# Russoul/cuda-mat

Measured on AMD Instinct MI355X. Metric: BiCGSTAB iters/sec + SpMV effective HBM GB/s, 10M-row CSR at 1/2/4/8 GPUs, higher is better.
Workload: dtype f64

## Files before the change

### cuda_mat_amd/csrc/config.cpp

```cpp
#include "config.h"

#include <stdio.h>
#include <stdlib.h>
#include <string.h>

#include <unistd.h>

#include <mutex>
#include <set>
#include <string>

extern char **environ;

#include "common.h"

namespace cm {

namespace {

enum Kind { K_FLAG, K_INT, K_LLONG, K_ENUM, K_FAIL };

struct Option {
    const char *name;
    Kind kind;
    int Config::*field;
    long long Config::*wide;
    long long lo, hi;
    const char *words;
    const char *help;
};

#define OPT_FLAG(NAME, FIELD, HELP) {NAME, K_FLAG, &Config::FIELD, nullptr, 0, 1, nullptr, HELP}
#define OPT_INT(NAME, FIELD, LO, HI, HELP) {NAME, K_INT, &Config::FIELD, nullptr, LO, HI, nullptr, HELP}
#define OPT_ENUM(NAME, FIELD, WORDS, HELP) {NAME, K_ENUM, &Config::FIELD, nullptr, 0, 0, WORDS, HELP}

const Option kOptions[] = {
    OPT_INT("VERBOSE", verbose, 0, 2, "1: set-up breakdowns and auto-tune timings on stderr; 2: also the memory classes of a large blocked copy's arrays (timed probe, diagnosis)"),
    OPT_FLAG("ROCTX", roctx, "roctx ranges around solver creation, SpMV-form choice, ILU(0) set-up, the loop, SpMVs and all-reduces"),
    OPT_ENUM("SPMV_MODE", spmv_mode, "csr=0,pb=1,sell=2,pat=3", "force the CSR forms / the blocked two-phase form / SELL-C-sigma / the row-pattern dictionary"),
    OPT_FLAG("SPMV_SELL", spmv_sell, "0: keep SELL-C-sigma out of the candidates"),
    OPT_ENUM("SPMV_FORM", spmv_form, "lanes=1,tiles=2", "inside the CSR forms: lanes per row / nnz-balanced tiles"),
    OPT_INT("SPMV_LANES", spmv_lanes, 2, 64, "lanes per row, a power of two (and no stream tiles)"),
    OPT_FLAG("SPMV_COMPRESS", spmv_compress, "0: stream kernel on the plain 32-bit indices"),
    OPT_FLAG("SPMV_ALIGN", spmv_align, "0: compressed stream kernel without line-aligned copies of its value / offset streams"),
    OPT_ENUM("SPMV_TUNE", spmv_tune_full, "full=1", "time every SpMV candidate even when the column span already decides"),
    OPT_FLAG("VALUE_DICT", value_dict, "0: keep fp64 values even when the matrix has <= 256 distinct ones"),
    OPT_INT("PB_MIN_WAVES", pb_min_waves, 256, 1 << 20, "blocked form: fewest phase-2 waves"),
    OPT_INT("PB_DEPTH", pb_depth, 4, 16, "blocked form: segment loads in flight per phase-2 wave (4, 8 or 16)"),
    OPT_FLAG("POOL", pool, "0: device memory straight from hipMalloc / hipFree instead of the library's recycling pool (read once per process)"),
    OPT_FLAG("SKIP_ORIG_COPY", skip_orig_copy, "0: cudamat_solve with ILU(0) builds the blocked copy in the original index space even when its loop will run in the level-major spaces"),
    OPT_FLAG("EARLY_ANALYSIS", early_analysis, "0: cudamat_solve analyses the ILU(0) levels after the upload of the values instead of beside it"),
    OPT_INT("PB_FILL_OCC", pb_fill_occ, 0, 64, "resident waves per CU of the two-pass fill's first pass (0: 8; probing)"),
    OPT_FLAG("PB_FILL2", pb_fill2, "0: fill the blocked copy with the single-pass scatter kernel (rounds 1-4) instead of the two-pass partition"),
    OPT_INT("PB_PLACE", pb_place, 0, 2, "blocked copy of a large matrix: 1 (default): a resident solver's product stream is placed in a memory class of its own, values and indices in another (timed probe of the device's memory classes, 10-35 ms per copy: spmv_pb.hip); 2: the drop-in calls place theirs as well; 0: arrays wherever the allocator puts them"),
    OPT_INT("PB_PLACE_MAX_MS", pb_place_max_ms, 0, 60000, "PB_PLACE: what the search for an arrangement may take before the arrays are allocated as ever (ms; the slabs it allocates included -- 0.3 ms per 16 GB on most boxes, 2 s on some)"),
    OPT_FLAG("PB_PROBE_FAIL", pb_probe_fail, "1 (tests): treat the run-time LDS-order probe as failed, i.e. select the architected-order phase 2"),
    OPT_FLAG("PB_STRICT", pb_strict, "1: phase 2 adds a row's products of one wave instruction rank by rank (architected order, +10 %)"),
    {"FUSED", K_LLONG, nullptr, &Config::fused, 0, 1LL << 40, nullptr,
     "0: never fold the vector updates into the SpMVs (three launches per iteration); N: do it for every supported plan up to N rows"},
    OPT_FLAG("RESIDENT", resident, "0: never run the whole loop of a very small system in one launch"),
    OPT_INT("RESIDENT_SPIN_LIMIT", resident_spin_limit, 0, 1 << 30, "polls a grid-barrier wait of the single-launch loop may take"),
    OPT_FLAG("GUARD", guard, "1: every solve on the context runs as if CUDAMAT_FLAG_GUARD were set: restart from the true residual when rho has lost its last bit, converged = 1 only for a verified iterate (reference loops, one GPU)"),
    {"GUARD_RHO_ULPS", K_LLONG, nullptr, &Config::guard_rho_ulps, 1, 1LL << 52, nullptr,
     "guarded solves restart when |rho| <= N * 2^-52 * sum |rw_i r_i| (default 4; 2^52 fires at every iteration >= 1: tests)"},
    OPT_INT("PIPE_RR", pipe_rr, 0, 1 << 20, "residual replacement period of the pipelined loop (0: never)"),
    OPT_FLAG("TRSV_SYNCFREE", trsv_syncfree, "0: one launch per level; 1: dependency-driven launches also for narrow levels"),
    OPT_FLAG("TRSV_LDS", trsv_lds, "0: no single-workgroup LDS-resident triangular solve for small systems"),
    OPT_FLAG("TRSV_HYBRID", trsv_hybrid, "0 | 1: never / always split big factors into far (blocked SpMV) and near (dependency-driven) parts"),
    OPT_INT("TRSV_GROUPS", trsv_groups, 2, 128, "groups of levels of a hybrid factor"),
    OPT_INT("TRSV_LANES", trsv_lanes, 2, 64, "lanes per row of the triangular-solve kernels, a power of two"),
    OPT_INT("TRSV_SPIN_LIMIT", trsv_spin_limit, 1, 1 << 30, "polls of one dependency before a row gives up"),
    OPT_FLAG("TRSV_PERM", trsv_perm, "0: permute around every M^-1 application instead of running the loop in the level-major spaces"),
    OPT_FLAG("LEVELS_SWEEP", levels_sweep, "1: level analysis by relaxation sweeps"),
    OPT_FLAG("ILU0_SIMPLE", ilu0_simple, "1: numeric ILU(0) without LDS staging / prefetch"),
    OPT_FLAG("FORCE_SHARDED", force_sharded, "1: keep the collective path at world size 1"),
    OPT_FLAG("OVERLAP", overlap, "0: plain all-gather instead of pieces behind phase 1 of the blocked SpMV"),
    OPT_INT("OVERLAP_CHUNKS", overlap_chunks, 1, 16, "pieces per slice of an overlapped gather"),
    OPT_FLAG("WINDOWED", windowed, "0: never exchange windows (halo) only"),
    OPT_FLAG("SHARDED_ONE_DEVICE", sharded_one_device,
             "1: cudamat_solve_sharded with every rank on device 0 and host-synchronised copies in place of RCCL (debugging aid)"),
    OPT_FLAG("PLAN_CACHE", plan_cache, "0: cudamat_solve does not keep the solver of its last call"),
    OPT_FLAG("ILU0_REFACTOR", ilu0_refactor, "0: cudamat_solve with ILU(0) on a reused plan whose factors belong to another shift repeats the whole ILU(0) set-up instead of the numeric-only refactorisation (cudamat_solver_ilu0_refactor)"),
    OPT_ENUM("MANY_FORM", many_form, "auto=0,batched=1,columns=2",
             "several right-hand sides: batched (one SpMM per step for up to 8 columns) / columns (one solve per column); auto: the faster as timed at the first solve"),
    OPT_ENUM("MANY_PRECOND", many_precond, "columns=0,auto=1,batched=2",
             "several right-hand sides with ILU(0): columns (one preconditioned solve per column, default) / batched (multi-column triangular solves and one SpMM per step for up to 8 columns, where the factors are covered) / auto: the faster as timed at the first such solve; MANY_FORM = columns overrides.  Governs cudamat_solver_solve_shifts_ilu0 (one set of ILU(0) factors per column) the same way: columns = one factorisation and one solve per column, batched = the K-wide factorisation and triangular solves with per-column values, auto = both timed with their factorisations"),
    {"TEST_COMM_FAIL", K_FAIL, nullptr, nullptr, 0, 0, nullptr, "rank:k -- fault injection: that rank's k-th all-reduce reports an error (tests)"},
};

bool power_of_two(long long v) { return v > 0 && (v & (v - 1)) == 0; }

bool apply(Config &cfg, const Option &o, const char *value)
{
    switch (o.kind) {
    case K_FLAG:
        if (!strcmp(value, "0") || !strcmp(value, "1")) { cfg.*(o.field) = value[0] - '0'; return true; }
        return false;
    case K_INT: {
        char *end = nullptr;
        const long long v = strtoll(value, &end, 10);
        if (end == value || *end || v < o.lo || v > o.hi) return false;
        if ((!strcmp(o.name, "SPMV_LANES") || !strcmp(o.name, "TRSV_LANES")) && !power_of_two(v)) return false;
        if (!strcmp(o.name, "PB_DEPTH") && v != 4 && v != 8 && v != 16) return false;
        cfg.*(o.field) = (int)v;
        return true;
    }
    case K_LLONG: {
        char *end = nullptr;
        const long long v = strtoll(value, &end, 10);
        if (end == value || *end || v < o.lo || v > o.hi) return false;
        cfg.*(o.wide) = v;
        return true;
    }
    case K_ENUM: {
        const size_t len = strlen(value);
        for (const char *w = o.words; w && *w;) {
            const char *eq = strchr(w, '=');
            if ((size_t)(eq - w) == len && !strncmp(w, value, len)) { cfg.*(o.field) = atoi(eq + 1); return true; }
            const char *comma = strchr(eq, ',');
            w = comma ? comma + 1 : nullptr;
        }
        return false;
    }
    case K_FAIL: {
        int r = -1, k = -1;
        if (sscanf(value, "%d:%d", &r, &k) != 2 || r < 0 || k < 1) return false;
        cfg.fail_rank = r;
        cfg.fail_call = k;
        return true;
    }
    }
    return false;
}

}

bool Config::operator==(const Config &o) const
{
    for (const Option &q : kOptions) {
        if (q.field && this->*(q.field) != o.*(q.field)) return false;
        if (q.wide && this->*(q.wide) != o.*(q.wide)) return false;
    }
    return fail_rank == o.fail_rank && fail_call == o.fail_call;
}

bool config_set(Config &cfg, const char *name, const char *value)
{
    if (!name || !value) { set_error("option name / value is NULL"); return false; }
    if (!strncmp(name, "CUDAMAT_", 8)) name += 8;
    for (const Option &o : kOptions) {
        if (strcmp(o.name, name)) continue;
        if (apply(cfg, o, value)) return true;
        set_error("option %s: value \"%s\" is not accepted (%s)", name, value, o.help);
        return false;
    }
    set_error("unknown option \"%s\" (cudamat_options_help lists them)", name);
    return false;
}

static void warn_once(const std::string &text)
{
    static std::mutex mu;
    static std::set<std::string> seen;
    std::lock_guard<std::mutex> lock(mu);
    if (seen.insert(text).second) fprintf(stderr, "cudamat: %s\n", text.c_str());
}

Config config_from_env()
{
    Config cfg;
    for (const Option &o : kOptions) {
        const std::string var = std::string("CUDAMAT_") + o.name;
        const char *v = getenv(var.c_str());
        if (!v || !*v) continue;
        if (!apply(cfg, o, v))
            warn_once(var + "=\"" + v + "\" is not an accepted value and was IGNORED (" + o.help + ")");
    }
    for (char **e = environ; e && *e; e++) {
        if (strncmp(*e, "CUDAMAT_", 8) || !strncmp(*e, "CUDAMAT_BENCH_", 14)) continue;
        const char *eq = strchr(*e, '=');
        if (!eq || !eq[1]) continue;
        const std::string name(*e + 8, (size_t)(eq - (*e + 8)));
        bool known = false;
        for (const Option &o : kOptions) known = known || name == o.name;
        if (!known) warn_once("CUDAMAT_" + name + " names no switch of this library and was IGNORED (cudamat_options_help lists them)");
    }
    return cfg;
}

const char *config_help()
{
    static const std::string text = [] {
        std::string t;
        for (const Option &o : kOptions) {
            t += "CUDAMAT_";
            t += o.name;
            t += o.kind == K_FLAG ? " = 0 | 1" : o.kind == K_ENUM ? " = " : o.kind == K_FAIL ? " = rank:k" : " = N";
            if (o.kind == K_ENUM) {
                for (const char *w = o.words; w && *w;) {
                    const char *eq = strchr(w, '=');
                    if (w != o.words) t += " | ";
                    t.append(w, (size_t)(eq - w));
                    const char *comma = strchr(eq, ',');
                    w = comma ? comma + 1 : nullptr;
                }
            }
            if (o.kind == K_INT || o.kind == K_LLONG) t += " in [" + std::to_string(o.lo) + ", " + std::to_string(o.hi) + "]";
            t += "   ";
            t += o.help;
            t += "\n";
        }
        return t;
    }();
    return text.c_str();
}

}
```

### cuda_mat_amd/csrc/config.h

```cpp
#pragma once

namespace cm {

struct Config {
    int verbose = 0;
    int roctx = 0;
    int spmv_mode = -1;
    int spmv_sell = 1;
    int spmv_form = 0;
    int spmv_lanes = 0;
    int spmv_compress = 1;
    int spmv_align = 1;
    int spmv_tune_full = 0;
    int value_dict = 1;
    int pb_min_waves = 0;
    int pb_depth = 0;
    int pool = 1;
    int skip_orig_copy = 1;
    int early_analysis = 1;
    int pb_fill_occ = 0;
    int pb_fill2 = 1;
    int pb_place = 1;
    int pb_place_max_ms = 300;
    int pb_probe_fail = 0;
    int pb_strict = 0;
    long long fused = -1;
    int resident = 1;
    int resident_spin_limit = -1;
    int guard = 0;
    long long guard_rho_ulps = 4;
    int pipe_rr = -1;
    int trsv_syncfree = -1;
    int trsv_lds = 1;
    int trsv_hybrid = -1;
    int trsv_groups = 0;
    int trsv_lanes = 0;
    int trsv_spin_limit = 0;
    int trsv_perm = 1;
    int levels_sweep = 0;
    int ilu0_simple = 0;
    int force_sharded = 0;
    int overlap = 1;
    int overlap_chunks = 0;
    int windowed = 1;
    int sharded_one_device = 0;
    int plan_cache = 1;
    int ilu0_refactor = 1;
    int many_form = 0;
    int many_precond = 0;
    int fail_rank = -1, fail_call = -1;

    bool operator==(const Config &o) const;
    bool operator!=(const Config &o) const { return !(*this == o); }
};

Config config_from_env();
bool config_set(Config &cfg, const char *name, const char *value);
const char *config_help();

}
```

### cuda_mat_amd/csrc/spmv_pb.h

```cpp
#pragma once
#include "kernels.h"
#include "valdict.h"

namespace cm {

constexpr int kPbMaxChunks = 16;

struct PbCols {
    int64_t per = 0;
    int chunks = 1;
    int rank = 0;
};

struct PbPlan {
    int n = 0;
    int64_t n_cols = 0;
    int64_t nnz = 0;
    int CB = 0, NCB = 0;
    int64_t per = 0;
    int chunks = 1;
    int64_t chunk_len = 0;
    int bpc = 0;
    int RB = 0, NRB = 0;
    int NW = 0;
    int SR = 0;
    int LPS = 64;
    int depth = 4;
    int NSUB = 0;
    double *pv = nullptr;
    unsigned char *pvi = nullptr;
    const double *dict = nullptr;
    int ndict = 0;
    unsigned short *pc = nullptr;
    unsigned short *pr = nullptr;
    double *P = nullptr;
    int *cstart = nullptr;
    int *col0 = nullptr;
    int *sstart = nullptr;
    int *slen = nullptr;
    int *order = nullptr;
    int part_off[kPbMaxChunks + 2] = {0};
    int placed = -1;
    int place_slabs = 0;
    double place_seconds = 0.0;
    float place_check_ms = 0.f, place_fast_ms = 0.f, place_slow_ms = 0.f;
    char place_classes[192] = {0};
    bool pc_zeroed = false;
    double build_seconds = 0.0;
};

struct PbCut {
    int per, chunks, chunk_len, bpc, CB;
};
struct PbBuild {
    PbPlan p;
    int *bins = nullptr;
    PbCut cut{};
    size_t cap = 0;
    double t0 = 0.0;
    bool verbose = false;
    bool two_pass = false;
    int place = 0;
    bool report_classes = false;
    double place_max_seconds = 0.3;
    int fill_occ = 0;
    int GB = 1, NG = 1;
    unsigned long long *smeta = nullptr;
    int *gstart = nullptr;
};
int pb_build_begin(hipStream_t st, const Config &cfg, int n, int64_t n_cols, int64_t nnz, const int *rp, const int *ci,
                   const PbCols *cols, PbBuild *b);
int pb_build_alloc(hipStream_t st, const Config &cfg, int n, int64_t n_cols, int64_t nnz, const PbCols *cols, PbBuild *b);
int pb_build_count(hipStream_t st, const Config &cfg, const int *rp, const int *ci, PbBuild *b);
int pb_build_values(hipStream_t st, PbBuild *b, const ValDict *vd);
int pb_build_fill(hipStream_t st, PbBuild *b, const int *rp, const int *ci, const double *val, const ValDict *vd, int sub0, int sub1);
int pb_build_end(hipStream_t st, PbBuild *b, PbPlan *out);
void pb_build_abort(PbBuild *b);

bool pb_candidate(hipStream_t st, int n, int64_t n_cols, int64_t nnz, const int *rp, const int *ci);
int pb_build(hipStream_t st, const Config &cfg, int n, int64_t n_cols, int64_t nnz, const int *rp, const int *ci,
             const double *val, PbPlan *out, const PbCols *cols = nullptr, const ValDict *vd = nullptr);
void pb_free(PbPlan *p);
int pb_strict_for(cudamat_ctx *ctx, int *strict);
int launch_spmv_pb(hipStream_t st, const PbPlan &plan, const SpmvArgs &a);
int launch_pb_check(hipStream_t st, const SpmvArgs &a);
int launch_pb_phase1(hipStream_t st, const PbPlan &plan, const SpmvArgs &a, int part);
int launch_pb_phase2(hipStream_t st, const PbPlan &plan, const SpmvArgs &a);

}
```

### cuda_mat_amd/csrc/spmv_pb.hip

```cpp
#include <algorithm>
#include <map>
#include <mutex>
#include <string>
#include <vector>

#include "device.h"
#include "spmv_pb.h"

namespace cm {

typedef unsigned short u16;
constexpr int kPbBuildWaves = 4;
constexpr int kP1Threads = 1024;
constexpr int kP1Unroll = 8;
constexpr int kTileMax = 13312;
constexpr int kPbAlign = 64;

void pb_free(PbPlan *p)
{
    void *ptrs[] = {p->pv, p->pvi, p->pc, p->pr, p->P, p->cstart, p->col0, p->sstart, p->slen, p->order};
    for (void *q : ptrs)
        if (q) CM_DROP(hipFree(q));
    *p = PbPlan();
}
// ... 324 lines not shown
}

__global__ __launch_bounds__(kBlock) void k_pb_segscan(int NCB, int NSUB, const int *cstart, int *bins, int *sstart,
                                                       int *slen)
{
    __shared__ int lds_waves[kBlock / 64];
    const int c = blockIdx.x;
    int *b = bins + (size_t)c * NSUB;
    int run = cstart[c];
    for (int s0 = 0; s0 < NSUB; s0 += kBlock) {
        const int sidx = s0 + threadIdx.x;
        const int cnt = sidx < NSUB ? b[sidx] : 0;
        int total;
        const int ex = block_scan_int(cnt, lds_waves, &total);
        if (sidx < NSUB) {
            const int start = run + ex;
            b[sidx] = start;
            sstart[(size_t)sidx * NCB + c] = start;
            slen[(size_t)sidx * NCB + c] = cnt;
        }
        run += total;
    }
}

static int round_blocks(int64_t n, int tile_max)
{
    int64_t m = (n + (int64_t)256 * tile_max - 1) / ((int64_t)256 * tile_max);
    if (m < 1) m = 1;
    return (int)(256 * m);
}

static void pb_scratch_free(PbBuild *b)
{
    if (b->smeta) CM_DROP(hipFree(b->smeta));
    if (b->gstart) CM_DROP(hipFree(b->gstart));
    b->smeta = nullptr;
    b->gstart = nullptr;
}

void pb_build_abort(PbBuild *b)
{
    pb_scratch_free(b);
    if (b->bins) CM_DROP(hipFree(b->bins));
    b->bins = nullptr;
    pb_free(&b->p);
}

int pb_build_begin(hipStream_t st, const Config &cfg, int n, int64_t n_cols, int64_t nnz, const int *rp, const int *ci,
                   const PbCols *cols, PbBuild *b)
{
    CM_TRY(pb_build_alloc(st, cfg, n, n_cols, nnz, cols, b));
    return pb_build_count(st, cfg, rp, ci, b);
}

int pb_build_alloc(hipStream_t st, const Config &cfg, int n, int64_t n_cols, int64_t nnz, const PbCols *cols, PbBuild *b)
{
    b->t0 = now_s();
    PbPlan &p = b->p;
    p = PbPlan();
    p.n = n;
    p.n_cols = n_cols;
    p.nnz = nnz;
    int local_slice = 0;
    if (cols && cols->per > 0 && cols->per < n_cols) {
        p.per = cols->per;
        p.chunks = cols->chunks < 1 ? 1 : cols->chunks > kPbMaxChunks ? kPbMaxChunks : cols->chunks;
        p.chunk_len = (p.per + p.chunks - 1) / p.chunks;
        p.bpc = (int)((p.chunk_len + kTileMax - 1) / kTileMax);
        p.CB = (int)((p.chunk_len + p.bpc - 1) / p.bpc);
        const int64_t slices = (n_cols + p.per - 1) / p.per;
        p.NCB = (int)(slices * p.chunks * p.bpc);
        local_slice = cols->rank;
    } else {
        p.per = n_cols;
        p.chunks = 1;
        p.chunk_len = n_cols;
        p.NCB = round_blocks(n_cols, kTileMax);
        p.CB = (int)((n_cols + p.NCB - 1) / p.NCB);
        p.NCB = (int)((n_cols + p.CB - 1) / p.CB);
        p.bpc = p.NCB;
    }
    const double seg_target = 48.0;
    double nsub_t = (double)nnz / ((double)p.NCB * seg_target);
    const bool few = nsub_t < 2560.0 && (double)n / 2048.0 * 8.0 * 8.0 <= 144.0 * 1024.0;
    double min_waves = few ? 2048.0 : 4096.0;
    if (cfg.pb_min_waves) min_waves = (double)cfg.pb_min_waves;
    if (nsub_t < min_waves) nsub_t = min_waves;
    if (nsub_t > (double)n / 16.0) nsub_t = (double)n / 16.0;
    if (nsub_t < 4.0) nsub_t = 4.0;
    p.NW = nsub_t >= 4096.0 ? 16 : nsub_t >= 2048.0 ? 8 : 4;
    int nrb = (int)(nsub_t / p.NW / 256.0 + 0.5) * 256;
    if (nrb < 256) nrb = 256;
    const int nrb_min = (int)(((int64_t)n + kTileMax - 1) / kTileMax);
    while (nrb < nrb_min) nrb += 256;
    if (nrb > kMaxParts) nrb = kMaxParts;
    p.NRB = nrb;
    p.RB = (int)(((int64_t)n + p.NRB - 1) / p.NRB);
    p.SR = (p.RB + p.NW - 1) / p.NW;
    if (p.SR < 1) p.SR = 1;
    p.RB = p.SR * p.NW;
    p.NRB = (int)(((int64_t)n + p.RB - 1) / p.RB);
    p.NSUB = p.NRB * p.NW;
    const double seg = (double)nnz / ((double)p.NCB * p.NSUB);
    p.LPS = seg <= 6.0 ? 16 : seg <= 22.0 ? 32 : 64;
    p.depth = few ? 16 : 4;
    if (cfg.pb_depth) p.depth = cfg.pb_depth;
    if (p.NRB > kMaxParts || p.CB > 65536 || p.SR > 65536 || (size_t)p.RB * 8 > 150 * 1024 ||
        sizeof(int) * (size_t)kPbBuildWaves * p.NCB > 150 * 1024) {
        set_error("pb_build: matrix shape outside the blocked kernel's limits");
        return CUDAMAT_ERR_ARG;
    }
    const size_t nbins = (size_t)p.NCB * p.NSUB;
    int *&bins = b->bins;
    bins = nullptr;
    int rc = CUDAMAT_OK;
    do {
        if ((rc = dev_alloc(&bins, nbins))) break;
        constexpr int align = kPbAlign;
        const size_t cap = (size_t)nnz + (size_t)(align - 1) * (size_t)p.NCB + 16;
        b->cap = cap;
        if ((rc = dev_alloc(&p.cstart, (size_t)p.NCB + 1))) break;
        if ((rc = dev_alloc(&p.col0, (size_t)p.NCB + 1))) break;
        if ((rc = dev_alloc(&p.order, (size_t)p.NCB))) break;
        {
            std::vector<int> h0((size_t)p.NCB + 1), ord;
            const int per_slice = p.chunks * p.bpc;
            for (int cb = 0; cb <= p.NCB; cb++) {
                const int64_t q = cb / per_slice, ch = (cb % per_slice) / p.bpc, k = cb % p.bpc;
                int64_t in_piece = k * (int64_t)p.CB;
                if (in_piece > p.chunk_len) in_piece = p.chunk_len;
                int64_t in_slice = ch * p.chunk_len + in_piece;
                if (in_slice > p.per) in_slice = p.per;
                int64_t c0 = q * p.per + in_slice;
                if (c0 > n_cols) c0 = n_cols;
                h0[(size_t)cb] = (int)c0;
            }
            ord.reserve((size_t)p.NCB);
            const int slices = p.NCB / per_slice;
            if (slices > 1) {
                for (int k = 0; k < per_slice; k++) ord.push_back(local_slice * per_slice + k);
                p.part_off[0] = 0;
                p.part_off[1] = (int)ord.size();
                for (int ch = 0; ch < p.chunks; ch++) {
                    for (int q = 0; q < slices; q++)
                        if (q != local_slice)
                            for (int k = 0; k < p.bpc; k++) ord.push_back((q * p.chunks + ch) * p.bpc + k);
                    p.part_off[ch + 2] = (int)ord.size();
                }
            } else {
                for (int cb = 0; cb < p.NCB; cb++) ord.push_back(cb);
                p.part_off[0] = 0;
                for (int ch = 0; ch <= p.chunks; ch++) p.part_off[ch + 1] = p.NCB;
            }
            if (hipMemcpyAsync(p.col0, h0.data(), sizeof(int) * h0.size(), hipMemcpyHostToDevice, st) != hipSuccess ||
                hipMemcpyAsync(p.order, ord.data(), sizeof(int) * ord.size(), hipMemcpyHostToDevice, st) != hipSuccess ||
                hipStreamSynchronize(st) != hipSuccess) { rc = CUDAMAT_ERR_HIP; set_error("pb column cut upload failed"); break; }
        }
        b->cut = PbCut{(int)p.per, p.chunks, (int)p.chunk_len, p.bpc, p.CB};
        if ((rc = dev_alloc(&p.sstart, nbins))) break;
        if ((rc = dev_alloc(&p.slen, nbins))) break;
        if ((rc = set_max_lds((const void *)k_pb_count))) break;
        if ((rc = set_max_lds((const void *)k_pb_rows<true>))) break;
        b->GB = 1;
        while (b->GB * kPbGroups < p.NCB) b->GB *= 2;
        b->NG = (p.NCB + b->GB - 1) / b->GB;
        b->fill_occ = cfg.pb_fill_occ;
        b->place = cfg.pb_place;
        b->place_max_seconds = 1e-3 * cfg.pb_place_max_ms;
        b->verbose = cfg.verbose != 0;
        b->report_classes = cfg.verbose >= 2;
        b->two_pass = cfg.pb_fill2 != 0 && nnz > 0 && nnz < 0x7fffffffLL && p.SR <= 65536 && b->GB <= 64;
        if (b->two_pass) {
            if (dev_alloc(&b->smeta, (size_t)nnz) != CUDAMAT_OK || dev_alloc(&b->gstart, (size_t)p.NSUB * (size_t)(b->NG + 1)) != CUDAMAT_OK) {
                if (b->smeta) CM_DROP(hipFree(b->smeta));
                b->smeta = nullptr;
                b->two_pass = false;
            }
        }
    } while (0);
    if (rc) pb_build_abort(b);
    return rc;
}

int pb_build_count(hipStream_t st, const Config &cfg, const int *rp, const int *ci, PbBuild *b)
{
    PbPlan &p = b->p;
    const int n = p.n;
    const int64_t nnz = p.nnz;
    int *bins = b->bins;
// ... 286 lines not shown
{
    PbPlan &p = b->p;
    const size_t cap = b->cap;
    const bool dict = vd && vd->n > 0;
    int rc = CUDAMAT_OK;
    if (dict && p.pv) {
        CM_DROP(hipFree(p.pv));
        p.pv = nullptr;
    }
    do {
        if (!p.P && b->place > 0 && sizeof(double) * cap >= kPlaceMinBytes) {
            void *v = nullptr, *c = nullptr, *r = nullptr, *pp = nullptr;
            bool placed = false;
            if ((rc = place_copy(st, b->verbose, b->place_max_seconds, dict ? cap : sizeof(double) * cap, sizeof(u16) * cap, sizeof(double) * cap, &v, &c, &r, &pp, &placed, &p))) break;
            if (placed) {
                if (dict) p.pvi = (unsigned char *)v; else p.pv = (double *)v;
                p.pc = (u16 *)c;
                p.pr = (u16 *)r;
                p.P = (double *)pp;
            }
        }
        if (dict) {
            if (!p.pvi && (rc = dev_alloc(&p.pvi, cap))) break;
            if (hipMemsetAsync(p.pvi, 0, cap, st) != hipSuccess) { rc = CUDAMAT_ERR_HIP; break; }
            p.dict = vd->dict;
            p.ndict = vd->n;
        } else {
            if (!p.pv && (rc = dev_alloc(&p.pv, cap))) break;
            if (hipMemsetAsync(p.pv, 0, sizeof(double) * cap, st) != hipSuccess) { rc = CUDAMAT_ERR_HIP; break; }
        }
        if (p.P && p.pc && p.pr && p.pc_zeroed) break;
        if (!p.pc && (rc = dev_alloc(&p.pc, cap))) break;
        if (!p.pr && (rc = dev_alloc(&p.pr, cap))) break;
        if (!p.P && (rc = dev_alloc(&p.P, cap))) break;
        if (kPbAlign > 1 && hipMemsetAsync(p.pc, 0, sizeof(u16) * cap, st) != hipSuccess) { rc = CUDAMAT_ERR_HIP; break; }
        p.pc_zeroed = true;
    } while (0);
    if (rc) pb_build_abort(b);
    return rc;
}

int pb_build_fill(hipStream_t st, PbBuild *b, const int *rp, const int *ci, const double *val, const ValDict *vd, int sub0, int sub1)
{
    PbPlan &p = b->p;
    if (sub1 > p.NSUB) sub1 = p.NSUB;
    if (sub1 <= sub0) return CUDAMAT_OK;
    const unsigned grid = (unsigned)((sub1 - sub0 + kPbBuildWaves - 1) / kPbBuildWaves);
    const unsigned char *vidx = p.pvi ? vd->idx : (const unsigned char *)nullptr;
    const int cfg_fill_occ = b->fill_occ;
    if (b->two_pass) {
        size_t pad = 0;
        if (cfg_fill_occ > 0) {
            const size_t per_wg = (size_t)(160 * 1024) / (size_t)((cfg_fill_occ + kPbBuildWaves - 1) / kPbBuildWaves);
            pad = per_wg > 40 * 1024 ? per_wg - 40 * 1024 : 0;
            if (pad > 64 * 1024) pad = 64 * 1024;
        }
        hipLaunchKernelGGL(k_pb_group, dim3(grid), dim3(64 * kPbBuildWaves), pad, st, p.n, rp, ci, val, vidx, b->cut, p.col0, p.NCB, p.SR,
                           p.slen, b->GB, b->NG, b->gstart, p.P, p.pvi ? (unsigned char *)p.P : (unsigned char *)nullptr, b->smeta, sub0, sub1);
        const long long buckets = (long long)(sub1 - sub0) * b->NG;
        hipLaunchKernelGGL(k_pb_scatter, dim3((unsigned)((buckets + kPbScatterWaves - 1) / kPbScatterWaves)), dim3(64 * kPbScatterWaves), 0, st,
                           p.NCB, p.NSUB, p.slen, b->bins, b->GB, b->NG, b->gstart, p.P, p.pvi ? (const unsigned char *)p.P : (const unsigned char *)nullptr,
                           b->smeta, p.pv, p.pvi, p.pc, p.pr, sub0, sub1);
    } else {
        const size_t lds = sizeof(int) * (size_t)kPbBuildWaves * p.NCB;
        hipLaunchKernelGGL(k_pb_rows<true>, dim3(grid), dim3(64 * kPbBuildWaves), lds, st, p.n, rp, ci, val, b->cut, p.col0,
                           p.NCB, p.SR, p.NSUB, b->bins, p.pv, p.pc, p.pr, vidx, p.pvi, sub0, sub1);
    }
    if (hipGetLastError() != hipSuccess) { set_error("pb fill launch failed"); pb_build_abort(b); return CUDAMAT_ERR_HIP; }
    return CUDAMAT_OK;
}

static void pb_print_plan(const PbPlan &p)
{
    const size_t nbins = (size_t)p.NCB * p.NSUB;
    std::vector<int> hl(nbins);
    if (hipMemcpy(hl.data(), p.slen, sizeof(int) * nbins, hipMemcpyDeviceToHost) != hipSuccess) return;
    long long hist[7] = {0, 0, 0, 0, 0, 0, 0}, in_long = 0;
    for (int v : hl) {
        hist[v == 0 ? 0 : v <= 8 ? 1 : v <= 24 ? 2 : v <= 48 ? 3 : v <= 64 ? 4 : v <= 128 ? 5 : 6]++;
        if (v > 64) in_long += v;
    }
    fprintf(stderr, "[cudamat] pb arrays: pv %p pvi %p pc %p pr %p P %p sstart %p slen %p cstart %p\n", (void *)p.pv, (void *)p.pvi, (void *)p.pc,
            (void *)p.pr, (void *)p.P, (void *)p.sstart, (void *)p.slen, (void *)p.cstart);
    fprintf(stderr, "[cudamat] pb plan: %d x %lld, nnz %lld, NCB %d (CB %d), NSUB %d (NW %d, SR %d), LPS %d, depth %d; segments: "
                    "empty %lld, 1-8 %lld, 9-24 %lld, 25-48 %lld, 49-64 %lld, 65-128 %lld, >128 %lld; %.1f %% of the entries in "
                    "segments longer than a wave\n",
            p.n, (long long)p.n_cols, (long long)p.nnz, p.NCB, p.CB, p.NSUB, p.NW, p.SR, p.LPS, p.depth, hist[0], hist[1], hist[2], hist[3],
            hist[4], hist[5], hist[6], 100.0 * (double)in_long / (double)(p.nnz > 0 ? p.nnz : 1));
}

static void place_report_classes(hipStream_t st, const PbPlan &p, size_t cap)
{
    if (!pool_enabled()) return;
    PlaceTimer tm(st);
    if (!tm.ok) return;
    int dev = 0;
    if (hipGetDevice(&dev) != hipSuccess) return;
    std::lock_guard<std::mutex> lock(g_place_mu);
    PlaceMemo &m = g_place[dev];
    if (m.gen != pool_generation()) { m.gen = pool_generation(); m.reset(); }
    std::vector<char *> slabs;
    std::vector<char *> scratch(3, nullptr);
    for (int k = 0; k < 4 && !(scratch[0] && scratch[1] && scratch[2]); k++) {
        char *base = nullptr;
        if (hipMalloc(&base, kPlaceSlab) != hipSuccess) { CM_DROP(hipGetLastError()); break; }
        slabs.push_back(base);
        char *seg = nullptr;
        size_t bytes = 0;
        if (!pool_segment_of(base, &seg, &bytes)) break;
        char *b0 = seg + ((size_t)(base - seg) + kPlaceBlock - 1) / kPlaceBlock * kPlaceBlock;
        for (char *q = b0; q + kPlaceBlock <= base + bytes; q += kPlaceBlock) {
            const int c = place_class_of(tm, m, q);
            if (c >= 0 && c < 3 && !scratch[c]) scratch[c] = q;
        }
    }
    struct Arr { const char *name; const char *ptr; size_t bytes; };
    const Arr arrs[4] = {{"values", p.pv ? (const char *)p.pv : (const char *)p.pvi, p.pv ? sizeof(double) * cap : cap},
                         {"col idx", (const char *)p.pc, sizeof(u16) * cap}, {"row idx", (const char *)p.pr, sizeof(u16) * cap}, {"products", (const char *)p.P, sizeof(double) * cap}};
    for (const Arr &a : arrs) {
        std::string line;
        for (size_t off = 0; off + kPlaceSample <= a.bytes; off += kPlaceSample) {
            int cls = -1;
            float worst = 0.f;
            for (int k = 0; k < 3; k++) {
                if (!scratch[k]) continue;
                const float t = tm.ms(a.ptr + off, scratch[k] + kPlaceBlock - kPlaceSample, kPlaceSample);
                if (t > worst) { worst = t; cls = k; }
            }
            line += cls < 0 || !(m.t_hi >= kPlaceGap * m.t_lo) || worst <= sqrtf(m.t_lo * m.t_hi) ? '?' : (char)('0' + cls);
        }
        fprintf(stderr, "[cudamat] pb classes: %-8s at %p, per %zu MB: %s\n", a.name, (const void *)a.ptr, kPlaceSample >> 20, line.c_str());
    }
    for (char *q : slabs) CM_DROP(hipFree(q));
}

int pb_build_end(hipStream_t st, PbBuild *b, PbPlan *out)
{
    if (hipStreamSynchronize(st) != hipSuccess) { set_error("pb fill failed"); pb_build_abort(b); return CUDAMAT_ERR_HIP; }
    if (b->verbose) pb_print_plan(b->p);
    if (b->report_classes && sizeof(double) * b->cap >= kPlaceMinBytes) place_report_classes(st, b->p, b->cap);
    pb_scratch_free(b);
    CM_DROP(hipFree(b->bins));
    b->bins = nullptr;
    b->p.build_seconds = now_s() - b->t0;
    *out = b->p;
    b->p = PbPlan();
    return CUDAMAT_OK;
}

int pb_build(hipStream_t st, const Config &cfg, int n, int64_t n_cols, int64_t nnz, const int *rp, const int *ci,
             const double *val, PbPlan *out, const PbCols *cols, const ValDict *vd)
{
    PbBuild b;
    CM_TRY(pb_build_begin(st, cfg, n, n_cols, nnz, rp, ci, cols, &b));
    CM_TRY(pb_build_values(st, &b, vd));
    CM_TRY(pb_build_fill(st, &b, rp, ci, val, vd, 0, b.p.NSUB));
    return pb_build_end(st, &b, out);
}


__global__ __launch_bounds__(kP1Threads) void k_pb_phase1(const double *x, const int *col0, const int *list,
                                                          const int *cstart, const double *pv, const u16 *pc,
                                                          double *P, const LoopState *st, int cb0)
{
    extern __shared__ __attribute__((aligned(16))) double xs[];
    if (st && st->state != 0) return;
    const int cb = list ? list[blockIdx.x] : (int)blockIdx.x + cb0;
    const int s = cstart[cb], e = cstart[cb + 1];
    if (s >= e) return;
    const int c0 = col0[cb], cn = col0[cb + 1] - c0;
// ... 36 lines not shown
                                                               const LoopState *st, int cb0)
{
    extern __shared__ __attribute__((aligned(16))) double xs[];
    if (st && st->state != 0) return;
    const int cb = list ? list[blockIdx.x] : (int)blockIdx.x + cb0;
    const int s = cstart[cb], e = cstart[cb + 1];
    if (s == e) return;
    double *dv = xs + cb_doubles;
    const int c0 = col0[cb], cn = col0[cb + 1] - c0;
    for (int i = threadIdx.x; i < cn; i += kP1Threads) xs[i] = x[c0 + i];
    if (threadIdx.x < kDictMax) dv[threadIdx.x] = dict[threadIdx.x];
    __syncthreads();
    constexpr int U = kP1Unroll, STEP = 2 * kP1Threads, CH = U * STEP;
    const int a0 = (s + 1) & ~1;
    if (threadIdx.x == 0 && s < a0) P[s] = dv[pvi[s]] * xs[pc[s]];
    int kb = a0;
    const int t2 = 2 * (int)threadIdx.x;
    for (; kb + CH <= e; kb += CH) {
        const int k = kb + t2;
        u16 iv[U];
        unsigned cv[U];
#pragma unroll
        for (int u = 0; u < U; u++) {
            iv[u] = *(const u16 *)(pvi + k + u * STEP);
            cv[u] = *(const unsigned *)(pc + k + u * STEP);
        }
#pragma unroll
        for (int u = 0; u < U; u++) {
            double2 o;
            o.x = dv[iv[u] & 0xffu] * xs[cv[u] & 0xffffu];
            o.y = dv[iv[u] >> 8] * xs[cv[u] >> 16];
            *(double2 *)(P + k + u * STEP) = o;
        }
    }
    {
        const int m = e > kb ? (e - kb) / STEP : 0;
        const int k = kb + t2;
        u16 iv[U - 1];
        unsigned cv[U - 1];
#pragma unroll
        for (int u = 0; u < U - 1; u++) {
            if (u < m) {
                iv[u] = *(const u16 *)(pvi + k + u * STEP);
                cv[u] = *(const unsigned *)(pc + k + u * STEP);
            }
        }
#pragma unroll
        for (int u = 0; u < U - 1; u++) {
            if (u < m) {
                double2 o;
                o.x = dv[iv[u] & 0xffu] * xs[cv[u] & 0xffffu];
                o.y = dv[iv[u] >> 8] * xs[cv[u] >> 16];
                *(double2 *)(P + k + u * STEP) = o;
            }
        }
        const int kr = k + m * STEP;
        if (kr + 1 < e) {
            const u16 iw = *(const u16 *)(pvi + kr);
            const unsigned cw = *(const unsigned *)(pc + kr);
            double2 o;
            o.x = dv[iw & 0xffu] * xs[cw & 0xffffu];
            o.y = dv[iw >> 8] * xs[cw >> 16];
            *(double2 *)(P + kr) = o;
        } else if (kr < e) {
            P[kr] = dv[pvi[kr]] * xs[pc[kr]];
        }
    }
}

struct Pb2Args {
    int n, NCB, SR;
    const int *sstart, *slen;
    const double *P;
    const u16 *pr;
    const double *d, *xd;
    double alpha, beta;
    double *y;
    int dot;
    const double *w;
    double *parts;
    const LoopState *st;
    int strict;
    const int *xd_idx;
};

__device__ __forceinline__ void pb_seg_add(double *my, int r, double p, bool on, int lane, int group_first, bool strict)
{
    if (!strict) {
        if (on) unsafeAtomicAdd(&my[r], p);
        return;
    }
    const int r_prev = __shfl_up(r, 1, 64);
    const int on_prev = __shfl_up((int)on, 1, 64);
    const bool d1 = on && lane > group_first && on_prev && r_prev == r;
    if (on && !d1) unsafeAtomicAdd(&my[r], p);
    if (__ballot(d1) == 0) return;
    const bool d2 = d1 && __shfl_up((int)d1, 1, 64) != 0;
    if (d1 && !d2) unsafeAtomicAdd(&my[r], p);
    if (__ballot(d2) == 0) return;
    int head = d1 ? 0 : lane;
#pragma unroll
    for (int o = 1; o < 64; o <<= 1) {
        const int t = __shfl_up(head, o, 64);
        if (lane >= o) head = t > head ? t : head;
    }
    const int rank = on ? lane - head : 0;
    for (int q = 2; __ballot(on && rank >= q); q++)
        if (on && rank == q) unsafeAtomicAdd(&my[r], p);
}

__global__ __launch_bounds__(64) void k_lds_order_probe(int *mismatch)
{
    __shared__ double acc[64], val[64], start[64];
    const int lane = threadIdx.x;
    unsigned long long z = 0x9E3779B97F4A7C15ULL * (unsigned long long)(lane + 1);
    int bad = 0;
    for (int pat = 0; pat < 4; pat++) {
        const int addr = pat == 0 ? 0 : pat == 1 ? lane >> 3 : pat == 2 ? (lane & 31) : (lane & 3);
        const int naddr = pat == 0 ? 1 : pat == 1 ? 8 : pat == 2 ? 32 : 4;
        for (int rep = 0; rep < 4; rep++) {
            z ^= z >> 30; z *= 0xBF58476D1CE4E5B9ULL; z ^= z >> 27; z *= 0x94D049BB133111EBULL; z ^= z >> 31;
            const double v = 0.5 + (double)(z >> 11) * 0x1.0p-53;
            const double c = 3.0 + (double)((z * 0x9E3779B97F4A7C15ULL) >> 11) * 0x1.0p-53;
            val[lane] = v;
            start[lane] = c;
            acc[lane] = c;
            __syncthreads();
            unsafeAtomicAdd(&acc[addr], v);
            __syncthreads();
            if (lane < naddr) {
#pragma clang fp contract(off)
                double e = start[lane];
                for (int l = 0; l < 64; l++) {
                    const int al = pat == 0 ? 0 : pat == 1 ? l >> 3 : pat == 2 ? (l & 31) : (l & 3);
                    if (al == lane) e = e + val[l];
                }
                if (__double_as_longlong(e) != __double_as_longlong(acc[lane])) bad = 1;
            }
            __syncthreads();
        }
    }
    if (bad) atomicOr(mismatch, 1);
}

int pb_strict_for(cudamat_ctx *ctx, int *strict)
{
    *strict = 1;
    if (ctx->cfg.pb_strict) return CUDAMAT_OK;
    if (ctx->lds_lane_order < 0) {
        int *flag = (int *)ctx->scratch.get(), h = 1;
        CM_HIP(hipMemsetAsync(flag, 0, sizeof(int), ctx->stream));
        hipLaunchKernelGGL(k_lds_order_probe, dim3(1), dim3(64), 0, ctx->stream, flag);
        CM_HIP(hipGetLastError());
        CM_HIP(hipMemcpyAsync(&h, flag, sizeof(int), hipMemcpyDeviceToHost, ctx->stream));
        CM_HIP(hipStreamSynchronize(ctx->stream));
        if (ctx->cfg.pb_probe_fail) h = 1;
        ctx->lds_lane_order = h ? 0 : 1;
        if (h || ctx->cfg.verbose)
            fprintf(stderr, "[cudamat] LDS order probe: equal addresses of one ds_add_f64 are %s -> blocked SpMV phase 2 in its %s form\n",
                    h ? (ctx->cfg.pb_probe_fail ? "reported NOT in lane order (PB_PROBE_FAIL)" : "NOT served in lane order")
                      : "served in lane order", h ? "architected-order (PB_STRICT)" : "default");
    }
    *strict = ctx->lds_lane_order ? 0 : 1;
    return CUDAMAT_OK;
}

template <int NW, int LPS, int DEPTH, bool IDX = false>
__global__ __launch_bounds__(64 * NW) void k_pb_phase2(Pb2Args a)
{
    extern __shared__ __attribute__((aligned(16))) double yt[];
    if (a.st && a.st->state != 0) return;
    const int wave = threadIdx.x >> 6, lane = threadIdx.x & 63;
    const int sub = blockIdx.x * NW + wave;
    double *my = yt + (size_t)wave * a.SR;
    for (int i = lane; i < a.SR; i += 64) my[i] = 0.0;
    __builtin_amdgcn_fence(__ATOMIC_RELEASE, "wavefront");
    __builtin_amdgcn_wave_barrier();
    const int *ss = a.sstart + (size_t)sub * a.NCB;
    const int *sl = a.slen + (size_t)sub * a.NCB;
    for (int cb0 = 0; cb0 < a.NCB; cb0 += 64) {
        const int c = cb0 + lane;
        const int mys = c < a.NCB ? ss[c] : 0;
        const int myl = c < a.NCB ? sl[c] : 0;
        const int lim = a.NCB - cb0 < 64 ? a.NCB - cb0 : 64;
        const bool grouped = LPS < 64 && !__any(myl > LPS);
        if (!grouped) {
            for (int j = 0; j < lim; j += DEPTH) {
                int s[DEPTH], l[DEPTH];
                double pv4[DEPTH];
                int r4[DEPTH];
#pragma unroll
                for (int u = 0; u < DEPTH; u++) {
                    s[u] = __builtin_amdgcn_readlane(mys, (j + u) & 63);
                    l[u] = __builtin_amdgcn_readlane(myl, (j + u) & 63);
                }
#pragma unroll
                for (int u = 0; u < DEPTH; u++) {
                    const bool on = lane < l[u];
                    pv4[u] = on ? a.P[s[u] + lane] : 0.0;
                    r4[u] = on ? (int)a.pr[s[u] + lane] : 0;
                }
#pragma unroll
                for (int u = 0; u < DEPTH; u++) {
                    pb_seg_add(my, r4[u], pv4[u], lane < l[u], lane, 0, a.strict != 0);
                    for (int off0 = 64; off0 < l[u]; off0 += 64) {
                        const int off = off0 + lane;
                        const bool on = off < l[u];
                        pb_seg_add(my, on ? (int)a.pr[s[u] + off] : 0, on ? a.P[s[u] + off] : 0.0, on, lane, 0, a.strict != 0);
                    }
                }
            }
        } else {
            constexpr int G = 64 / LPS;
            const int g = lane / LPS, li = lane % LPS;
            for (int j = 0; j < lim; j += DEPTH * G) {
                int s[DEPTH], l[DEPTH];
                double pv4[DEPTH];
                int r4[DEPTH];
#pragma unroll
                for (int u = 0; u < DEPTH; u++) {
                    const int cbi = j + u * G + g;
                    s[u] = __shfl(mys, cbi & 63, 64);
                    l[u] = cbi < 64 ? __shfl(myl, cbi & 63, 64) : 0;
                }
#pragma unroll
                for (int u = 0; u < DEPTH; u++) {
                    const bool on = li < l[u];
                    pv4[u] = on ? a.P[s[u] + li] : 0.0;
                    r4[u] = on ? (int)a.pr[s[u] + li] : 0;
                }
#pragma unroll
                for (int u = 0; u < DEPTH; u++) {
                    if (!a.strict) {
                        if (li < l[u]) unsafeAtomicAdd(&my[r4[u]], pv4[u]);
                    } else {
#pragma unroll
                        for (int gg = 0; gg < G; gg++)
                            pb_seg_add(my, r4[u], pv4[u], g == gg && li < l[u], lane, gg * LPS, true);
                    }
                }
            }
        }
    }
    __builtin_amdgcn_fence(__ATOMIC_RELEASE, "wavefront");
    __builtin_amdgcn_wave_barrier();
    double acc0 = 0.0, acc1 = 0.0;
    const long long row0 = (long long)sub * a.SR;
    for (int i = lane; i < a.SR && row0 + i < a.n; i += 64) {
#pragma clang fp contract(off)
        const int row = (int)(row0 + i);
        double sum = my[i];
        if (a.d) {
            const double dx = a.d[row] * a.xd[IDX ? a.xd_idx[row] : row];
            sum = sum + dx;
        }
        double out = a.alpha * sum;
        if (a.beta != 0.0) {
            const double by = a.beta * a.y[row];
            out = out + by;
        }
        a.y[row] = out;
        if (a.dot) {
            acc0 += out * a.w[row];
            acc1 += out * out;
        }
    }
    if (a.dot) {
        double *red = yt + (size_t)NW * a.SR;
#pragma unroll
        for (int o = 32; o > 0; o >>= 1) {
            acc0 += __shfl_xor(acc0, o, 64);
            acc1 += __shfl_xor(acc1, o, 64);
        }
        if (lane == 0) {
            red[2 * wave] = acc0;
            red[2 * wave + 1] = acc1;
        }
        __syncthreads();
        if (threadIdx.x == 0) {
            double t0 = 0.0, t1 = 0.0;
            for (int q = 0; q < NW; q++) {
                t0 += red[2 * q];
                t1 += red[2 * q + 1];
            }
            a.parts[2 * blockIdx.x] = t0;
            a.parts[2 * blockIdx.x + 1] = t1;
        }
    }
}

int launch_pb_check(hipStream_t st, const SpmvArgs &a)
{
    if (a.loop.st && a.check == CHECK_HALF) CM_TRY(launch_check(st, a.loop, a.half, CHECK_HALF));
    return CUDAMAT_OK;
}

static int launch_pb_phase1_blocks(hipStream_t st, const PbPlan &p, const SpmvArgs &a, const int *list, int first, int last)
{
    if (last <= first) return CUDAMAT_OK;
    if (p.pvi) {
        CM_TRY(set_max_lds((const void *)k_pb_phase1_dict));
        const int cbd = (p.CB + 1) & ~1;
        hipLaunchKernelGGL(k_pb_phase1_dict, dim3(last - first), dim3(kP1Threads), sizeof(double) * (size_t)(cbd + kDictMax), st, a.x,
                           p.col0, list ? list + first : (const int *)nullptr, p.cstart, p.pvi, p.pc, p.dict, cbd, p.P, a.loop.st,
                           list ? 0 : first);
        CM_HIP(hipGetLastError());
        return CUDAMAT_OK;
    }
    CM_TRY(set_max_lds((const void *)k_pb_phase1));
    hipLaunchKernelGGL(k_pb_phase1, dim3(last - first), dim3(kP1Threads), sizeof(double) * (size_t)p.CB, st, a.x, p.col0,
                       list ? list + first : (const int *)nullptr, p.cstart, p.pv, p.pc, p.P, a.loop.st, list ? 0 : first);
    CM_HIP(hipGetLastError());
    return CUDAMAT_OK;
}

int launch_pb_phase1(hipStream_t st, const PbPlan &p, const SpmvArgs &a, int part)
{
    if (part < 0) return launch_pb_phase1_blocks(st, p, a, nullptr, 0, p.NCB);
    return launch_pb_phase1_blocks(st, p, a, p.order, p.part_off[part], p.part_off[part + 1]);
}

int launch_spmv_pb(hipStream_t st, const PbPlan &p, const SpmvArgs &a)
{
    CM_TRY(launch_pb_check(st, a));
    CM_TRY(launch_pb_phase1(st, p, a, -1));
    return launch_pb_phase2(st, p, a);
}

int launch_pb_phase2(hipStream_t st, const PbPlan &p, const SpmvArgs &a)
{
    Pb2Args b;
    b.n = p.n; b.NCB = p.NCB; b.SR = p.SR;
    b.sstart = p.sstart; b.slen = p.slen;
    b.P = p.P; b.pr = p.pr;
    b.d = a.d; b.xd = a.xd; b.xd_idx = a.xd_idx;
    b.alpha = a.alpha; b.beta = a.beta;
    b.y = a.y; b.dot = a.dot; b.w = a.w; b.parts = a.parts;
    b.st = a.loop.st;
    b.strict = a.pb_strict;
    const size_t lds = sizeof(double) * ((size_t)p.NW * p.SR + 2 * (size_t)p.NW);
    const bool idx = b.d && b.xd_idx;
#define CM_P2D(NWV, LPSV, DV, IDXV)                                                                               \
    do {                                                                                                          \
        CM_TRY(set_max_lds((const void *)k_pb_phase2<NWV, LPSV, DV, IDXV>));                                     \
        hipLaunchKernelGGL((k_pb_phase2<NWV, LPSV, DV, IDXV>), dim3(p.NRB), dim3(64 * NWV), lds, st, b);         \
    } while (0)
#define CM_P2(NWV, LPSV)                                                                                  \
    do {                                                                                                  \
        if (idx && p.depth >= 16) CM_P2D(NWV, LPSV, 16, true);                                            \
        else if (idx) CM_P2D(NWV, LPSV, 4, true);                                                         \
        else if (p.depth >= 16) CM_P2D(NWV, LPSV, 16, false);                                             \
        else if (p.depth >= 8) CM_P2D(NWV, LPSV, 8, false);                                               \
        else CM_P2D(NWV, LPSV, 4, false);                                                                 \
    } while (0)
#define CM_P2_LPS(NWV)                                           \
    do {                                                         \
        if (p.LPS == 16) CM_P2(NWV, 16);                         \
        else if (p.LPS == 32) CM_P2(NWV, 32);                    \
        else CM_P2(NWV, 64);                                     \
    } while (0)
    switch (p.NW) {
    case 4:  CM_P2_LPS(4); break;
    case 8:  CM_P2_LPS(8); break;
    default: CM_P2_LPS(16); break;
    }
#undef CM_P2_LPS
#undef CM_P2
#undef CM_P2D
    CM_HIP(hipGetLastError());
    return CUDAMAT_OK;
}

}
```

Measured before the change: 184.0.

## Keep phase-2 waves in lockstep with periodic workgroup barriers on full matrices

Adds a lockstep option to the blocked SpMV phase 2, so the waves of a workgroup meet at an s_barrier every N column blocks. It is enabled by default (period 64, depth 8) for large full-shape plans. The aim is to keep the waves' streaming over column blocks aligned, so their x/product accesses share cache lines and DRAM pages instead of drifting apart. Barriers add stall time when waves are imbalanced, and the default depth for these plans changes from 4 to 8.

```diff
diff --git a/cuda_mat_amd/csrc/config.cpp b/cuda_mat_amd/csrc/config.cpp
--- a/cuda_mat_amd/csrc/config.cpp
+++ b/cuda_mat_amd/csrc/config.cpp
@@ -47,6 +47,7 @@
     OPT_FLAG("VALUE_DICT", value_dict, "0: keep fp64 values even when the matrix has <= 256 distinct ones"),
     OPT_INT("PB_MIN_WAVES", pb_min_waves, 256, 1 << 20, "blocked form: fewest phase-2 waves"),
     OPT_INT("PB_DEPTH", pb_depth, 4, 16, "blocked form: segment loads in flight per phase-2 wave (4, 8 or 16)"),
+    OPT_INT("PB_LOCKSTEP", pb_lockstep, 0, 64, "blocked form: the waves of a phase-2 workgroup meet at a barrier every N column blocks (16, 32 or 64; a multiple of depth x segments per wave instruction, else ignored for that plan); 0: never, and the former depth by shape (default: 64 with 8 loads in flight for a full matrix of >= 4096 waves with whole-wave segments, else never)"),
     OPT_FLAG("POOL", pool, "0: device memory straight from hipMalloc / hipFree instead of the library's recycling pool (read once per process)"),
     OPT_FLAG("SKIP_ORIG_COPY", skip_orig_copy, "0: cudamat_solve with ILU(0) builds the blocked copy in the original index space even when its loop will run in the level-major spaces"),
     OPT_FLAG("EARLY_ANALYSIS", early_analysis, "0: cudamat_solve analyses the ILU(0) levels after the upload of the values instead of beside it"),
@@ -102,6 +103,7 @@
         if (end == value || *end || v < o.lo || v > o.hi) return false;
         if ((!strcmp(o.name, "SPMV_LANES") || !strcmp(o.name, "TRSV_LANES")) && !power_of_two(v)) return false;
         if (!strcmp(o.name, "PB_DEPTH") && v != 4 && v != 8 && v != 16) return false;
+        if (!strcmp(o.name, "PB_LOCKSTEP") && v != 0 && v != 16 && v != 32 && v != 64) return false;
         cfg.*(o.field) = (int)v;
         return true;
     }
@@ -165,6 +167,8 @@
     std::lock_guard<std::mutex> lock(mu);
     if (seen.insert(text).second) fprintf(stderr, "cudamat: %s\n", text.c_str());
 }
+
+void config_warn_once(const char *text) { warn_once(text); }
 
 Config config_from_env()
 {
diff --git a/cuda_mat_amd/csrc/config.h b/cuda_mat_amd/csrc/config.h
--- a/cuda_mat_amd/csrc/config.h
+++ b/cuda_mat_amd/csrc/config.h
@@ -18,6 +18,7 @@
     int pool = 1;
     int skip_orig_copy = 1;
     int early_analysis = 1;
+    int pb_lockstep = -1;
     int pb_fill_occ = 0;
     int pb_fill2 = 1;
     int pb_place = 1;
@@ -57,5 +58,6 @@
 Config config_from_env();
 bool config_set(Config &cfg, const char *name, const char *value);
 const char *config_help();
+void config_warn_once(const char *text);
 
 }
diff --git a/cuda_mat_amd/csrc/spmv_pb.h b/cuda_mat_amd/csrc/spmv_pb.h
--- a/cuda_mat_amd/csrc/spmv_pb.h
+++ b/cuda_mat_amd/csrc/spmv_pb.h
@@ -26,6 +26,7 @@
     int SR = 0;
     int LPS = 64;
     int depth = 4;
+    int lockstep = 0;
     int NSUB = 0;
     double *pv = nullptr;
     unsigned char *pvi = nullptr;
diff --git a/cuda_mat_amd/csrc/spmv_pb.hip b/cuda_mat_amd/csrc/spmv_pb.hip
--- a/cuda_mat_amd/csrc/spmv_pb.hip
+++ b/cuda_mat_amd/csrc/spmv_pb.hip
@@ -430,6 +430,7 @@
     }
     const double seg_target = 48.0;
     double nsub_t = (double)nnz / ((double)p.NCB * seg_target);
+    const double nsub_natural = nsub_t;
     const bool few = nsub_t < 2560.0 && (double)n / 2048.0 * 8.0 * 8.0 <= 144.0 * 1024.0;
     double min_waves = few ? 2048.0 : 4096.0;
     if (cfg.pb_min_waves) min_waves = (double)cfg.pb_min_waves;
@@ -451,8 +452,22 @@
     p.NSUB = p.NRB * p.NW;
     const double seg = (double)nnz / ((double)p.NCB * p.NSUB);
     p.LPS = seg <= 6.0 ? 16 : seg <= 22.0 ? 32 : 64;
-    p.depth = few ? 16 : 4;
+    const bool full = nsub_natural >= 4096.0 && p.NW == 16 && p.LPS == 64;
+    p.depth = few ? 16 : full && cfg.pb_lockstep < 0 ? 8 : 4;
     if (cfg.pb_depth) p.depth = cfg.pb_depth;
+    p.lockstep = 0;
+    const int want_lockstep = cfg.pb_lockstep >= 0 ? cfg.pb_lockstep : full && !cfg.pb_depth ? 64 : 0;
+    if (want_lockstep > 0) {
+        const int group = p.depth * (64 / p.LPS);
+        if (want_lockstep % group == 0 && !(p.depth == 8 && p.LPS < 64)) p.lockstep = want_lockstep;
+        else {
+            char text[256];
+            snprintf(text, sizeof text, "CUDAMAT_PB_LOCKSTEP=\"%d\" was IGNORED for a blocked copy with depth %d and %d segments per wave "
+                     "instruction: a period is a multiple of their product, %d, and depth 8 takes one with whole-wave segments only",
+                     cfg.pb_lockstep, p.depth, 64 / p.LPS, group);
+            config_warn_once(text);
+        }
+    }
     if (p.NRB > kMaxParts || p.CB > 65536 || p.SR > 65536 || (size_t)p.RB * 8 > 150 * 1024 ||
         sizeof(int) * (size_t)kPbBuildWaves * p.NCB > 150 * 1024) {
         set_error("pb_build: matrix shape outside the blocked kernel's limits");
@@ -905,10 +920,10 @@
     }
     fprintf(stderr, "[cudamat] pb arrays: pv %p pvi %p pc %p pr %p P %p sstart %p slen %p cstart %p\n", (void *)p.pv, (void *)p.pvi, (void *)p.pc,
             (void *)p.pr, (void *)p.P, (void *)p.sstart, (void *)p.slen, (void *)p.cstart);
-    fprintf(stderr, "[cudamat] pb plan: %d x %lld, nnz %lld, NCB %d (CB %d), NSUB %d (NW %d, SR %d), LPS %d, depth %d; segments: "
+    fprintf(stderr, "[cudamat] pb plan: %d x %lld, nnz %lld, NCB %d (CB %d), NSUB %d (NW %d, SR %d), LPS %d, depth %d, lockstep %d; segments: "
                     "empty %lld, 1-8 %lld, 9-24 %lld, 25-48 %lld, 49-64 %lld, 65-128 %lld, >128 %lld; %.1f %% of the entries in "
                     "segments longer than a wave\n",
-            p.n, (long long)p.n_cols, (long long)p.nnz, p.NCB, p.CB, p.NSUB, p.NW, p.SR, p.LPS, p.depth, hist[0], hist[1], hist[2], hist[3],
+            p.n, (long long)p.n_cols, (long long)p.nnz, p.NCB, p.CB, p.NSUB, p.NW, p.SR, p.LPS, p.depth, p.lockstep, hist[0], hist[1], hist[2], hist[3],
             hist[4], hist[5], hist[6], 100.0 * (double)in_long / (double)(p.nnz > 0 ? p.nnz : 1));
 }
 
@@ -1111,6 +1126,7 @@
     const LoopState *st;
     int strict;
     const int *xd_idx;
+    int period;
 };
 
 __device__ __forceinline__ void pb_seg_add(double *my, int r, double p, bool on, int lane, int group_first, bool strict)
@@ -1194,7 +1210,7 @@
     return CUDAMAT_OK;
 }
 
-template <int NW, int LPS, int DEPTH, bool IDX = false>
+template <int NW, int LPS, int DEPTH, bool IDX = false, bool LOCK = false>
 __global__ __launch_bounds__(64 * NW) void k_pb_phase2(Pb2Args a)
 {
     extern __shared__ __attribute__((aligned(16))) double yt[];
@@ -1207,69 +1223,76 @@
     __builtin_amdgcn_wave_barrier();
     const int *ss = a.sstart + (size_t)sub * a.NCB;
     const int *sl = a.slen + (size_t)sub * a.NCB;
+    const int period = DEPTH >= 16 ? 64 : a.period;
     for (int cb0 = 0; cb0 < a.NCB; cb0 += 64) {
         const int c = cb0 + lane;
         const int mys = c < a.NCB ? ss[c] : 0;
         const int myl = c < a.NCB ? sl[c] : 0;
         const int lim = a.NCB - cb0 < 64 ? a.NCB - cb0 : 64;
         const bool grouped = LPS < 64 && !__any(myl > LPS);
-        if (!grouped) {
-            for (int j = 0; j < lim; j += DEPTH) {
-                int s[DEPTH], l[DEPTH];
-                double pv4[DEPTH];
-                int r4[DEPTH];
-#pragma unroll
-                for (int u = 0; u < DEPTH; u++) {
-                    s[u] = __builtin_amdgcn_readlane(mys, (j + u) & 63);
-                    l[u] = __builtin_amdgcn_readlane(myl, (j + u) & 63);
-                }
-#pragma unroll
-                for (int u = 0; u < DEPTH; u++) {
-                    const bool on = lane < l[u];
-                    pv4[u] = on ? a.P[s[u] + lane] : 0.0;
-                    r4[u] = on ? (int)a.pr[s[u] + lane] : 0;
-                }
-#pragma unroll
-                for (int u = 0; u < DEPTH; u++) {
-                    pb_seg_add(my, r4[u], pv4[u], lane < l[u], lane, 0, a.strict != 0);
-                    for (int off0 = 64; off0 < l[u]; off0 += 64) {
-                        const int off = off0 + lane;
-                        const bool on = off < l[u];
-                        pb_seg_add(my, on ? (int)a.pr[s[u] + off] : 0, on ? a.P[s[u] + off] : 0.0, on, lane, 0, a.strict != 0);
+        int j0 = 0;
+        do {
+            const int j1 = LOCK && j0 + period < lim ? j0 + period : lim;
+            if (LOCK) __builtin_amdgcn_s_barrier();
+            if (!grouped) {
+                for (int j = j0; j < j1; j += DEPTH) {
+                    int s[DEPTH], l[DEPTH];
+                    double pv4[DEPTH];
+                    int r4[DEPTH];
+#pragma unroll
+                    for (int u = 0; u < DEPTH; u++) {
+                        s[u] = __builtin_amdgcn_readlane(mys, (j + u) & 63);
+                        l[u] = __builtin_amdgcn_readlane(myl, (j + u) & 63);
+                    }
+#pragma unroll
+                    for (int u = 0; u < DEPTH; u++) {
+                        const bool on = lane < l[u];
+                        pv4[u] = on ? a.P[s[u] + lane] : 0.0;
+                        r4[u] = on ? (int)a.pr[s[u] + lane] : 0;
+                    }
+#pragma unroll
+                    for (int u = 0; u < DEPTH; u++) {
+                        pb_seg_add(my, r4[u], pv4[u], lane < l[u], lane, 0, a.strict != 0);
+                        for (int off0 = 64; off0 < l[u]; off0 += 64) {
+                            const int off = off0 + lane;
+                            const bool on = off < l[u];
+                            pb_seg_add(my, on ? (int)a.pr[s[u] + off] : 0, on ? a.P[s[u] + off] : 0.0, on, lane, 0, a.strict != 0);
+                        }
                     }
                 }
-            }
-        } else {
-            constexpr int G = 64 / LPS;
-            const int g = lane / LPS, li = lane % LPS;
-            for (int j = 0; j < lim; j += DEPTH * G) {
-                int s[DEPTH], l[DEPTH];
-                double pv4[DEPTH];
-                int r4[DEPTH];
-#pragma unroll
-                for (int u = 0; u < DEPTH; u++) {
-                    const int cbi = j + u * G + g;
-                    s[u] = __shfl(mys, cbi & 63, 64);
-                    l[u] = cbi < 64 ? __shfl(myl, cbi & 63, 64) : 0;
-                }
-#pragma unroll
-                for (int u = 0; u < DEPTH; u++) {
-                    const bool on = li < l[u];
-                    pv4[u] = on ? a.P[s[u] + li] : 0.0;
-                    r4[u] = on ? (int)a.pr[s[u] + li] : 0;
-                }
-#pragma unroll
-                for (int u = 0; u < DEPTH; u++) {
-                    if (!a.strict) {
-                        if (li < l[u]) unsafeAtomicAdd(&my[r4[u]], pv4[u]);
-                    } else {
-#pragma unroll
-                        for (int gg = 0; gg < G; gg++)
-                            pb_seg_add(my, r4[u], pv4[u], g == gg && li < l[u], lane, gg * LPS, true);
+            } else {
+                constexpr int G = 64 / LPS;
+                const int g = lane / LPS, li = lane % LPS;
+                for (int j = j0; j < j1; j += DEPTH * G) {
+                    int s[DEPTH], l[DEPTH];
+                    double pv4[DEPTH];
+                    int r4[DEPTH];
+#pragma unroll
+                    for (int u = 0; u < DEPTH; u++) {
+                        const int cbi = j + u * G + g;
+                        s[u] = __shfl(mys, cbi & 63, 64);
+                        l[u] = cbi < 64 ? __shfl(myl, cbi & 63, 64) : 0;
+                    }
+#pragma unroll
+                    for (int u = 0; u < DEPTH; u++) {
+                        const bool on = li < l[u];
+                        pv4[u] = on ? a.P[s[u] + li] : 0.0;
+                        r4[u] = on ? (int)a.pr[s[u] + li] : 0;
+                    }
+#pragma unroll
+                    for (int u = 0; u < DEPTH; u++) {
+                        if (!a.strict) {
+                            if (li < l[u]) unsafeAtomicAdd(&my[r4[u]], pv4[u]);
+                        } else {
+#pragma unroll
+                            for (int gg = 0; gg < G; gg++)
+                                pb_seg_add(my, r4[u], pv4[u], g == gg && li < l[u], lane, gg * LPS, true);
+                        }
                     }
                 }
             }
-        }
+            j0 += period;
+        } while (LOCK && j0 < lim);
     }
     __builtin_amdgcn_fence(__ATOMIC_RELEASE, "wavefront");
     __builtin_amdgcn_wave_barrier();
@@ -1369,10 +1392,16 @@
     b.strict = a.pb_strict;
     const size_t lds = sizeof(double) * ((size_t)p.NW * p.SR + 2 * (size_t)p.NW);
     const bool idx = b.d && b.xd_idx;
+    b.period = p.lockstep;
+#define CM_P2L(NWV, LPSV, DV, IDXV, LOCKV)                                                                              \
+    do {                                                                                                                \
+        CM_TRY(set_max_lds((const void *)k_pb_phase2<NWV, LPSV, DV, IDXV, LOCKV>));                                    \
+        hipLaunchKernelGGL((k_pb_phase2<NWV, LPSV, DV, IDXV, LOCKV>), dim3(p.NRB), dim3(64 * NWV), lds, st, b);        \
+    } while (0)
 #define CM_P2D(NWV, LPSV, DV, IDXV)                                                                               \
     do {                                                                                                          \
-        CM_TRY(set_max_lds((const void *)k_pb_phase2<NWV, LPSV, DV, IDXV>));                                     \
-        hipLaunchKernelGGL((k_pb_phase2<NWV, LPSV, DV, IDXV>), dim3(p.NRB), dim3(64 * NWV), lds, st, b);         \
+        if (p.lockstep > 0) CM_P2L(NWV, LPSV, DV, IDXV, (DV != 8 || LPSV == 64));                                 \
+        else CM_P2L(NWV, LPSV, DV, IDXV, false);                                                                  \
     } while (0)
 #define CM_P2(NWV, LPSV)                                                                                  \
     do {                                                                                                  \
@@ -1396,6 +1425,7 @@
 #undef CM_P2_LPS
 #undef CM_P2
 #undef CM_P2D
+#undef CM_P2L
     CM_HIP(hipGetLastError());
     return CUDAMAT_OK;
 }
```

After: 185.0, median of 6. About the same (+0.6%).
